# SamsungLabs/nb-asr

Hardware: AMD Instinct MI355X
Metric: utterances_per_sec (higher is better)
Workload: dtype f32

## Files before the change

### nb_asr_amd/csrc/layernorm.hip

```cpp
#include "storage.h"

namespace nbasr {

constexpr int LN_ROWS = 16;
constexpr int LN_QS = 16;

template <typename T, bool MINMAX = false, int FR = Chunk<T>::FR>
__device__ __forceinline__ void tile_statistics(const T* x, int channels, int ld, float eps, size_t base, bool active,
                                                int row, int ql, float (*s_mean)[LN_QS * FR], float (*s_m2)[LN_QS * FR],
                                                float* s_cnt, float* s_mu, float* s_rstd,
                                                float (*s_lo)[LN_QS * FR] = nullptr, float (*s_hi)[LN_QS * FR] = nullptr)
{
    float shift[FR], s1[FR], s2[FR], lo[FR], hi[FR];
#pragma unroll
    for (int r = 0; r < FR; ++r) { shift[r] = 0.f; s1[r] = 0.f; s2[r] = 0.f; lo[r] = 3.0e38f; hi[r] = -3.0e38f; }
    int n = 0;
    if (active && row < channels) {
        load_frames<FR>(x + base + static_cast<size_t>(row) * ld, shift);
        auto fold = [&](const float (&e)[FR]) {
#pragma unroll
            for (int r = 0; r < FR; ++r) {
                const float d = e[r] - shift[r];
                s1[r] += d;
                s2[r] = __builtin_fmaf(d, d, s2[r]);
                if (MINMAX) { lo[r] = fminf(lo[r], e[r]); hi[r] = fmaxf(hi[r], e[r]); }
            }
            ++n;
        };
        int c = row;
        for (; c + 7 * LN_ROWS < channels; c += 8 * LN_ROWS) {
            float e[8][FR];
#pragma unroll
            for (int u = 0; u < 8; ++u) load_frames<FR>(x + base + static_cast<size_t>(c + u * LN_ROWS) * ld, e[u]);
#pragma unroll
            for (int u = 0; u < 8; ++u) fold(e[u]);
        }
        for (; c + 3 * LN_ROWS < channels; c += 4 * LN_ROWS) {
            float e[4][FR];
#pragma unroll
            for (int u = 0; u < 4; ++u) load_frames<FR>(x + base + static_cast<size_t>(c + u * LN_ROWS) * ld, e[u]);
#pragma unroll
            for (int u = 0; u < 4; ++u) fold(e[u]);
        }
        for (; c < channels; c += LN_ROWS) {
            float e[FR];
            load_frames<FR>(x + base + static_cast<size_t>(c) * ld, e);
            fold(e);
        }
    }
    const float fn = static_cast<float>(n);
#pragma unroll
    for (int r = 0; r < FR; ++r) {
        const float dm = n ? s1[r] / fn : 0.f;
        s_mean[row][ql * FR + r] = shift[r] + dm;
        s_m2[row][ql * FR + r] = n ? fmaxf(s2[r] - dm * s1[r], 0.f) : 0.f;
        if (MINMAX) { s_lo[row][ql * FR + r] = lo[r]; s_hi[row][ql * FR + r] = hi[r]; }
    }
    if (ql == 0) s_cnt[row] = fn;
    __syncthreads();

    if (threadIdx.x < LN_QS * FR) {
        const int col = threadIdx.x;
        float cnt = 0.f, mean = 0.f, m2 = 0.f;
#pragma unroll
        for (int k = 0; k < LN_ROWS; ++k) {
            const float nb = s_cnt[k];
            if (nb > 0.f) {
                const float tot = cnt + nb;
                const float delta = s_mean[k][col] - mean;
                mean += delta * (nb / tot);
                m2 += s_m2[k][col] + delta * delta * (cnt * nb / tot);
                cnt = tot;
            }
        }
        s_mu[col] = mean;
        s_rstd[col] = 1.0f / sqrtf(m2 / fmaxf(cnt, 1.f) + eps);
        if (MINMAX) {
            float l = s_lo[0][col], h = s_hi[0][col];
#pragma unroll
            for (int k = 1; k < LN_ROWS; ++k) { l = fminf(l, s_lo[k][col]); h = fmaxf(h, s_hi[k][col]); }
            s_lo[0][col] = l; s_hi[0][col] = h;
        }
    }
    __syncthreads();
}

template <typename TI, typename TO, bool ABSMAX>
__global__ __launch_bounds__(256) void layernorm_channels_kernel(
    const TI* x, const float* __restrict__ gamma, const float* __restrict__ beta,
    TO* y, int channels, int frames, int ld, float eps, unsigned* __restrict__ absmax)
{
    constexpr int FR = Chunk<TI>::FR;
    __shared__ float s_mean[LN_ROWS][LN_QS * FR];
    __shared__ float s_m2[LN_ROWS][LN_QS * FR];
    __shared__ float s_cnt[LN_ROWS];
    __shared__ float s_mu[LN_QS * FR];
    __shared__ float s_rstd[LN_QS * FR];

    const int ql = threadIdx.x & (LN_QS - 1);
    const int row = threadIdx.x / LN_QS;
    const int nq = ld / FR;
    const int q = blockIdx.x * LN_QS + ql;
    const int b = blockIdx.y;
    const bool active = q < nq;
    const size_t base = static_cast<size_t>(b) * channels * ld + static_cast<size_t>(q) * FR;

    tile_statistics<TI>(x, channels, ld, eps, base, active, row, ql, s_mean, s_m2, s_cnt, s_mu, s_rstd);

    if (!active && !ABSMAX) return;
    float mu[FR], rs[FR];
#pragma unroll
    for (int r = 0; r < FR; ++r) { mu[r] = s_mu[ql * FR + r]; rs[r] = s_rstd[ql * FR + r]; }
    const int t0 = q * FR;
    float amax = 0.f;
    for (int c = row; active && c < channels; c += LN_ROWS) {
        const size_t off = base + static_cast<size_t>(c) * ld;
        float o[FR];
        load_frames<FR>(x + off, o);
        const float g = gamma[c], bt = beta[c];
#pragma unroll
        for (int r = 0; r < FR; ++r) {
            o[r] = (o[r] - mu[r]) * rs[r] * g + bt;
            if (t0 + r >= frames) o[r] = 0.f;
            if (ABSMAX) amax = fmaxf(amax, finite_abs(o[r]));
        }
        store_frames<FR, false>(y + off, o);
    }
    if (ABSMAX) {
#pragma unroll
        for (int m = 32; m >= 1; m >>= 1) amax = fmaxf(amax, __shfl_xor(amax, m));
        if ((threadIdx.x & 63) == 0) atomicMax(absmax + b, __float_as_uint(amax));
    }
}

template <typename T>
__global__ __launch_bounds__(256) void channel_stats_kernel(const T* __restrict__ x, float* __restrict__ stats,
                                                            int channels, int frames, int ld, float eps)
{
    constexpr int FR = Chunk<T>::FR;
    __shared__ float s_mean[LN_ROWS][LN_QS * FR];
    __shared__ float s_m2[LN_ROWS][LN_QS * FR];
    __shared__ float s_cnt[LN_ROWS];
    __shared__ float s_mu[LN_QS * FR];
    __shared__ float s_rstd[LN_QS * FR];

    const int ql = threadIdx.x & (LN_QS - 1);
    const int row = threadIdx.x / LN_QS;
    const int nq = ld / FR;
    const int q = blockIdx.x * LN_QS + ql;
    const int b = blockIdx.y;
    const bool active = q < nq;
    const size_t base = static_cast<size_t>(b) * channels * ld + static_cast<size_t>(q) * FR;

    tile_statistics<T>(x, channels, ld, eps, base, active, row, ql, s_mean, s_m2, s_cnt, s_mu, s_rstd);

    if (threadIdx.x < LN_QS * FR) {
        const int t = blockIdx.x * (LN_QS * FR) + threadIdx.x;
        if (t < ld) {
            const bool live = t < frames;
            float* srow = stats + static_cast<size_t>(b) * 2 * ld;
            srow[t] = live ? s_mu[threadIdx.x] : 0.f;
            srow[ld + t] = live ? s_rstd[threadIdx.x] : 0.f;
        }
    }
}

}

using namespace nbasr;

static int layernorm_impl(const char* what, const void* x, const float* gamma, const float* beta, void* y, float* absmax,
                          int batch, int channels, int frames, int ld, float eps, nbasr_stream_t stream,
                          int in_dtype = NBASR_F32, int out_dtype = NBASR_F32)
{
    clear_error();
    NBASR_REQUIRE((in_dtype == NBASR_F32 || in_dtype == NBASR_BF16) && (out_dtype == NBASR_F32 || out_dtype == NBASR_BF16) &&
                  !(in_dtype == NBASR_F32 && out_dtype == NBASR_BF16), NBASR_EINVAL,
                  "%s: storage types (%d -> %d) unsupported (f32 -> f32, bf16 -> bf16, bf16 -> f32)", what, in_dtype, out_dtype);
    NBASR_REQUIRE(batch >= 0 && channels > 0 && frames >= 0, NBASR_EINVAL, "%s: bad sizes", what);
    const int fr = in_dtype == NBASR_BF16 ? 8 : 4;
    NBASR_REQUIRE(ld >= frames && ld % fr == 0, NBASR_EALIGN, "%s: ld=%d must be >= frames=%d and a multiple of %d", what, ld, frames, fr);
    if (batch == 0 || ld == 0) return NBASR_OK;
    NBASR_REQUIRE(x && gamma && beta && y, NBASR_ENULL, "%s: NULL pointer", what);
    NBASR_REQUIRE(aligned16(x) && aligned16(y), NBASR_EALIGN, "%s: x, y must be 16-byte aligned", what);
    NBASR_REQUIRE(batch <= 65535, NBASR_EINVAL, "%s: batch %d > 65535", what, batch);
    NBASR_REQUIRE(!absmax || in_dtype == NBASR_F32, NBASR_EINVAL, "%s: the absmax by-product exists for fp32 tensors only", what);
    const int nq = ld / fr;
    const dim3 grid((nq + LN_QS - 1) / LN_QS, batch);
    if (in_dtype == NBASR_BF16) {
        if (out_dtype == NBASR_BF16)
            hipLaunchKernelGGL((layernorm_channels_kernel<bf16_t, bf16_t, false>), grid, dim3(256), 0, as_stream(stream),
                               static_cast<const bf16_t*>(x), gamma, beta, static_cast<bf16_t*>(y), channels, frames, ld, eps, static_cast<unsigned*>(nullptr));
        else
            hipLaunchKernelGGL((layernorm_channels_kernel<bf16_t, float, false>), grid, dim3(256), 0, as_stream(stream),
                               static_cast<const bf16_t*>(x), gamma, beta, static_cast<float*>(y), channels, frames, ld, eps, static_cast<unsigned*>(nullptr));
    } else if (absmax) {
        zero_async(absmax, sizeof(float) * batch, as_stream(stream));
        hipLaunchKernelGGL((layernorm_channels_kernel<float, float, true>), grid, dim3(256), 0, as_stream(stream),
                           static_cast<const float*>(x), gamma, beta, static_cast<float*>(y), channels, frames, ld, eps, reinterpret_cast<unsigned*>(absmax));
    } else {
        hipLaunchKernelGGL((layernorm_channels_kernel<float, float, false>), grid, dim3(256), 0, as_stream(stream),
                           static_cast<const float*>(x), gamma, beta, static_cast<float*>(y), channels, frames, ld, eps, static_cast<unsigned*>(nullptr));
    }
    return launch_status(what);
}

extern "C" int nbasr_layernorm_channels(const void* x, const float* gamma, const float* beta, void* y, float* absmax, int batch,
                                        int channels, int frames, int ld, float eps, int in_dtype, int out_dtype, nbasr_stream_t stream)
{
    clear_error();
    NBASR_REQUIRE(!absmax || (in_dtype == NBASR_F32 && out_dtype == NBASR_F32), NBASR_EINVAL,
                  "nbasr_layernorm_channels: the max|y| by-product exists for fp32 -> fp32 only");
    return layernorm_impl("nbasr_layernorm_channels", x, gamma, beta, y, absmax, batch, channels, frames, ld, eps, stream, in_dtype, out_dtype);
}

__global__ __launch_bounds__(256) void channel_stats_bound_kernel(const float* __restrict__ x, const float* __restrict__ gamma,
                                                                  const float* __restrict__ beta, float* __restrict__ stats,
                                                                  unsigned* __restrict__ bound, int channels, int frames, int ld, float eps)
{
    __shared__ float s_mean[LN_ROWS][LN_QS * 4];
    __shared__ float s_m2[LN_ROWS][LN_QS * 4];
    __shared__ float s_cnt[LN_ROWS];
    __shared__ float s_mu[LN_QS * 4];
    __shared__ float s_rstd[LN_QS * 4];
    __shared__ float s_gb[8];
    __shared__ float s_lo[LN_ROWS][LN_QS * 4];
    __shared__ float s_hi[LN_ROWS][LN_QS * 4];

    const int ql = threadIdx.x & (LN_QS - 1);
    const int row = threadIdx.x / LN_QS;
    const int nq = ld >> 2;
    const int q = blockIdx.x * LN_QS + ql;
    const int b = blockIdx.y;
    const bool active = q < nq;
    const size_t base = static_cast<size_t>(b) * channels * ld + static_cast<size_t>(q) * 4;

    float gm = 0.f, bm = 0.f;
    for (int c = threadIdx.x; c < channels; c += 256) { gm = fmaxf(gm, fabsf(gamma[c])); bm = fmaxf(bm, fabsf(beta[c])); }
#pragma unroll
    for (int d = 32; d >= 1; d >>= 1) { gm = fmaxf(gm, __shfl_xor(gm, d)); bm = fmaxf(bm, __shfl_xor(bm, d)); }
    if ((threadIdx.x & 63) == 0) { s_gb[threadIdx.x >> 6] = gm; s_gb[4 + (threadIdx.x >> 6)] = bm; }

    tile_statistics<float, true>(x, channels, ld, eps, base, active, row, ql, s_mean, s_m2, s_cnt, s_mu, s_rstd, s_lo, s_hi);
    gm = fmaxf(fmaxf(s_gb[0], s_gb[1]), fmaxf(s_gb[2], s_gb[3]));
    bm = fmaxf(fmaxf(s_gb[4], s_gb[5]), fmaxf(s_gb[6], s_gb[7]));

    float dev = 0.f;
    if (threadIdx.x < LN_QS * 4) {
        const int t = blockIdx.x * (LN_QS * 4) + threadIdx.x;
        if (t < ld) {
            const bool live = t < frames;
            float* srow = stats + static_cast<size_t>(b) * 2 * ld;
            srow[t] = live ? s_mu[threadIdx.x] : 0.f;
            srow[ld + t] = live ? s_rstd[threadIdx.x] : 0.f;
            if (live) dev = finite_abs(fmaxf(s_hi[0][threadIdx.x] - s_mu[threadIdx.x], s_mu[threadIdx.x] - s_lo[0][threadIdx.x]) * s_rstd[threadIdx.x]);
        }
    }
    if (threadIdx.x < 64) {
#pragma unroll
        for (int d = 32; d >= 1; d >>= 1) dev = fmaxf(dev, __shfl_xor(dev, d));
        if (threadIdx.x == 0) atomicMax(bound + b, __float_as_uint(finite_abs((dev * gm + bm) * 1.0001f)));
    }
}

template <bool NORM>
__global__ __launch_bounds__(256) void normalize_split_kernel(const float* __restrict__ x, const float* __restrict__ stats,
                                                              const float* __restrict__ gamma, const float* __restrict__ beta,
                                                              const float* __restrict__ bound, unsigned char* __restrict__ image,
                                                              int channels, int , int ld,
                                                              int bound_stride)
{
    typedef _Float16 halfx8 __attribute__((ext_vector_type(8)));
    constexpr int SPLIT_PITCH = 68;
    __shared__ __attribute__((aligned(16))) unsigned char s_tile[4][2][4 * SPLIT_PITCH * 16];
    const int ql = threadIdx.x & 63, wv = threadIdx.x >> 6, oct0 = wv + 4 * blockIdx.z;
    const int nq = ld >> 2;
    const int q = blockIdx.x * 64 + ql;
    const int b = blockIdx.y;
    const int n_groups = (channels + 15) >> 4;
    const size_t rows = static_cast<size_t>(ld) + 1;
    unsigned char* const img_b = image + static_cast<size_t>(b) * n_groups * 4 * rows * 16;
    if (blockIdx.x == 0 && blockIdx.z == 0) {
        const uint4 z = make_uint4(0u, 0u, 0u, 0u);
        for (int pl = threadIdx.x; pl < n_groups * 4; pl += 256) *reinterpret_cast<uint4*>(img_b + static_cast<size_t>(pl) * rows * 16) = z;
    }
    if (blockIdx.x * 64 >= nq) return;
    const bool inside = q < nq;
    float scale = 1.f;
    {
        const unsigned bits = __float_as_uint(bound[static_cast<size_t>(b) * bound_stride]);
        const int e = static_cast<int>((bits >> 23) & 0xffu);
        int k = (bits & 0x7fffffffu) ? (127 + 14) - e : 0;
        k = k > 126 ? 126 : (k < -126 ? -126 : k);
        scale = __uint_as_float(static_cast<unsigned>(127 + k) << 23);
    }
    float m4[4] = {0.f, 0.f, 0.f, 0.f}, r4[4] = {0.f, 0.f, 0.f, 0.f};
    if constexpr (NORM) {
        if (inside) {
            const float* st = stats + static_cast<size_t>(b) * 2 * ld + q * 4;
            const float4 mu = *reinterpret_cast<const float4*>(st), rs = *reinterpret_cast<const float4*>(st + ld);
            m4[0] = mu.x; m4[1] = mu.y; m4[2] = mu.z; m4[3] = mu.w;
            r4[0] = rs.x; r4[1] = rs.y; r4[2] = rs.z; r4[3] = rs.w;
        }
    }
    const float* xb = x + static_cast<size_t>(b) * channels * ld + static_cast<size_t>(q) * 4;
    const int n_oct = (channels + 7) >> 3;
    const int oct_step = 4 * gridDim.z;
    auto load_octet = [&](int oct, float4 (&t)[8]) {
#pragma unroll
        for (int c = 0; c < 8; ++c) {
            const int ch = oct * 8 + c;
            t[c] = make_float4(0.f, 0.f, 0.f, 0.f);
            if (inside && oct < n_oct && ch < channels) t[c] = *reinterpret_cast<const float4*>(xb + static_cast<size_t>(ch) * ld);
        }
    };
    unsigned char* const tile_hi = s_tile[wv][0];
    unsigned char* const tile_lo = s_tile[wv][1];
    float4 cur[8];
    if (oct0 < 2 * n_groups) load_octet(oct0, cur);
    for (int oct = oct0; oct < 2 * n_groups; oct += oct_step) {
        float4 nxt[8];
        if (oct + oct_step < 2 * n_groups) load_octet(oct + oct_step, nxt);
        else {
#pragma unroll
            for (int c = 0; c < 8; ++c) nxt[c] = make_float4(0.f, 0.f, 0.f, 0.f);
        }
        float v[8][4];
#pragma unroll
        for (int c = 0; c < 8; ++c) {
            const int ch = oct * 8 + c;
            float g = 0.f, be = 0.f;
            if constexpr (NORM) {
                if (oct < n_oct && ch < channels) { g = gamma[ch]; be = beta[ch]; }
            }
            const float e4[4] = {cur[c].x, cur[c].y, cur[c].z, cur[c].w};
#pragma unroll
            for (int r = 0; r < 4; ++r) {
                if constexpr (NORM) v[c][r] = (ch < channels) ? ln_apply(e4[r], m4[r], r4[r], g, be) * scale : 0.f;
                else                v[c][r] = e4[r] * scale;
            }
        }
#pragma unroll
        for (int r = 0; r < 4; ++r) {
            halfx8 hi, lo;
#pragma unroll
            for (int c = 0; c < 8; ++c) {
                const _Float16 h = static_cast<_Float16>(v[c][r]);
                hi[c] = h;
                lo[c] = static_cast<_Float16>(v[c][r] - static_cast<float>(h));
            }
            *reinterpret_cast<halfx8*>(tile_hi + (r * SPLIT_PITCH + ql) * 16) = hi;
            *reinterpret_cast<halfx8*>(tile_lo + (r * SPLIT_PITCH + ql) * 16) = lo;
        }
        asm volatile("s_waitcnt lgkmcnt(0)" ::: "memory");
        unsigned char* plane_hi = img_b + ((static_cast<size_t>(oct >> 1) * 4 + (oct & 1)) * rows + 1 + static_cast<size_t>(blockIdx.x) * 256) * 16;
        unsigned char* plane_lo = plane_hi + 2 * rows * 16;
#pragma unroll
        for (int k = 0; k < 4; ++k) {
            const int src = ((ql & 3) * SPLIT_PITCH + 16 * k + (ql >> 2)) * 16;
            const halfx8 hi = *reinterpret_cast<const halfx8*>(tile_hi + src);
            const halfx8 lo = *reinterpret_cast<const halfx8*>(tile_lo + src);
            const int f = 64 * k + ql;
            if (blockIdx.x * 256 + f < ld) {
                *reinterpret_cast<halfx8*>(plane_hi + f * 16) = hi;
                *reinterpret_cast<halfx8*>(plane_lo + f * 16) = lo;
            }
        }
        asm volatile("s_waitcnt lgkmcnt(0)" ::: "memory");
#pragma unroll
        for (int c = 0; c < 8; ++c) cur[c] = nxt[c];
    }
}

static int split_grid_z(int tiles, int batch)
{
    const long long wgs = static_cast<long long>(tiles) * batch;
    int z = 4;
    while (z < 16 && wgs * z < 512) z *= 2;
    return z;
}

extern "C" int nbasr_layernorm_split_image(const float* x, const float* gamma, const float* beta, float* stats, float* bound,
                                           void* image, int batch, int channels, int frames, int ld, float eps,
                                           nbasr_stream_t stream)
{
    clear_error();
    NBASR_REQUIRE(batch >= 0 && channels > 0 && frames >= 0, NBASR_EINVAL, "nbasr_layernorm_split_image: bad sizes");
    NBASR_REQUIRE(ld >= frames && ld % 4 == 0, NBASR_EALIGN, "nbasr_layernorm_split_image: ld=%d must be >= frames=%d and a multiple of 4", ld, frames);
    if (batch == 0 || ld == 0) return NBASR_OK;
    NBASR_REQUIRE(x && gamma && beta && stats && bound && image, NBASR_ENULL, "nbasr_layernorm_split_image: NULL pointer");
    NBASR_REQUIRE(aligned16(x) && aligned16(stats) && aligned16(image), NBASR_EALIGN, "nbasr_layernorm_split_image: x, stats, image must be 16-byte aligned");
    NBASR_REQUIRE(batch <= 65535, NBASR_EINVAL, "nbasr_layernorm_split_image: batch %d > 65535", batch);
    zero_async(bound, sizeof(float) * batch, as_stream(stream));
    const int nq = ld / 4;
    hipLaunchKernelGGL(channel_stats_bound_kernel, dim3((nq + LN_QS - 1) / LN_QS, batch), dim3(256), 0, as_stream(stream),
                       x, gamma, beta, stats, reinterpret_cast<unsigned*>(bound), channels, frames, ld, eps);
    hipLaunchKernelGGL(normalize_split_kernel<true>, dim3((nq + 63) / 64, batch, split_grid_z((nq + 63) / 64, batch)), dim3(256), 0, as_stream(stream),
                       x, stats, gamma, beta, bound, static_cast<unsigned char*>(image), channels, frames, ld, 1);
    return launch_status("nbasr_layernorm_split_image");
}

__global__ __launch_bounds__(256) void input_range_kernel(const float* __restrict__ x, unsigned* __restrict__ range,
                                                          int channels, int frames, int ld)
{
    __shared__ float s_max[4][256];
    __shared__ unsigned s_bad[4];
    const int b = blockIdx.y;
    const int lane = threadIdx.x & 63, slice = threadIdx.x >> 6;
    const int t0 = (blockIdx.x * 64 + lane) * 4;
    float m[4] = {0.f, 0.f, 0.f, 0.f};
    unsigned bad = 0u;
    if (t0 < frames) {
        const float* col = x + static_cast<size_t>(b) * channels * ld + t0;
        const bool whole = t0 + 4 <= ld && ld % 4 == 0 && (reinterpret_cast<size_t>(x) & 15) == 0;
        for (int c = slice; c < channels; c += 4) {
            float v[4] = {0.f, 0.f, 0.f, 0.f};
            if (whole) {
                const float4 q = *reinterpret_cast<const float4*>(col + static_cast<size_t>(c) * ld);
                v[0] = q.x; v[1] = q.y; v[2] = q.z; v[3] = q.w;
            } else {
#pragma unroll
                for (int r = 0; r < 4; ++r) if (t0 + r < frames) v[r] = col[static_cast<size_t>(c) * ld + r];
            }
#pragma unroll
            for (int r = 0; r < 4; ++r) {
                const float a = fabsf(v[r]);
                if (t0 + r < frames) {
                    if (!(a <= 3.4028234664e38f)) bad = 1u;
                    else m[r] = fmaxf(m[r], a);
                }
            }
        }
    }
#pragma unroll
    for (int r = 0; r < 4; ++r) s_max[slice][lane * 4 + r] = m[r];
#pragma unroll
    for (int d = 32; d >= 1; d >>= 1) bad |= __shfl_xor(bad, d);
    if (lane == 0) s_bad[slice] = bad;
    __syncthreads();
    const int t = blockIdx.x * 256 + threadIdx.x;
    const float fmax_ = fmaxf(fmaxf(s_max[0][threadIdx.x], s_max[1][threadIdx.x]), fmaxf(s_max[2][threadIdx.x], s_max[3][threadIdx.x]));
    float hi = fmax_, lo = (t < frames && fmax_ > 0.f) ? fmax_ : __uint_as_float(0x7f800000u);
#pragma unroll
    for (int d = 32; d >= 1; d >>= 1) {
        hi = fmaxf(hi, __shfl_xor(hi, d));
        lo = fminf(lo, __shfl_xor(lo, d));
    }
    if (lane == 0) {
        atomicMax(range + 4 * b, __float_as_uint(hi));
        atomicMin(range + 4 * b + 1, __float_as_uint(lo));
        if (slice == 0 && (s_bad[0] | s_bad[1] | s_bad[2] | s_bad[3])) atomicOr(range + 4 * b + 2, 0x3f800000u);
    }
}

__global__ void input_range_init_kernel(unsigned* __restrict__ range, int batch)
{
    const int b = blockIdx.x * blockDim.x + threadIdx.x;
    if (b < batch) { range[4 * b] = 0u; range[4 * b + 1] = 0x7f800000u; range[4 * b + 2] = 0u; range[4 * b + 3] = 0u; }
}

extern "C" int nbasr_input_range(const float* x, float* range, int batch, int channels, int frames, int ld, nbasr_stream_t stream)
{
    clear_error();
    NBASR_REQUIRE(batch >= 0 && channels > 0 && frames >= 0 && ld >= frames, NBASR_EINVAL, "nbasr_input_range: bad sizes");
    if (batch == 0) return NBASR_OK;
    NBASR_REQUIRE(range, NBASR_ENULL, "nbasr_input_range: range is NULL");
    NBASR_REQUIRE(batch <= 65535, NBASR_EINVAL, "nbasr_input_range: batch %d > 65535", batch);
    hipLaunchKernelGGL(input_range_init_kernel, dim3((batch + 255) / 256), dim3(256), 0, as_stream(stream), reinterpret_cast<unsigned*>(range), batch);
    if (frames > 0) {
        NBASR_REQUIRE(x, NBASR_ENULL, "nbasr_input_range: x is NULL");
        hipLaunchKernelGGL(input_range_kernel, dim3((frames + 255) / 256, batch), dim3(256), 0, as_stream(stream), x,
                           reinterpret_cast<unsigned*>(range), channels, frames, ld);
    }
    return launch_status("nbasr_input_range");
}

extern "C" int nbasr_split_image_ranged(const float* x, const float* x_range, void* image, int batch, int channels, int frames,
                                        int ld, nbasr_stream_t stream)
{
    clear_error();
    NBASR_REQUIRE(batch >= 0 && channels > 0 && frames >= 0, NBASR_EINVAL, "nbasr_split_image_ranged: bad sizes");
    NBASR_REQUIRE(ld >= frames && ld % 4 == 0, NBASR_EALIGN, "nbasr_split_image_ranged: ld=%d must be >= frames=%d and a multiple of 4", ld, frames);
    if (batch == 0 || ld == 0) return NBASR_OK;
    NBASR_REQUIRE(x && x_range && image, NBASR_ENULL, "nbasr_split_image_ranged: NULL pointer");
    NBASR_REQUIRE(aligned16(x) && aligned16(image), NBASR_EALIGN, "nbasr_split_image_ranged: x, image must be 16-byte aligned");
    NBASR_REQUIRE(batch <= 65535, NBASR_EINVAL, "nbasr_split_image_ranged: batch %d > 65535", batch);
    const int nq = ld / 4;
    hipLaunchKernelGGL(normalize_split_kernel<false>, dim3((nq + 63) / 64, batch, split_grid_z((nq + 63) / 64, batch)), dim3(256), 0, as_stream(stream),
                       x, static_cast<const float*>(nullptr), static_cast<const float*>(nullptr), static_cast<const float*>(nullptr),
                       x_range, static_cast<unsigned char*>(image), channels, frames, ld, 4);
    return launch_status("nbasr_split_image_ranged");
}

extern "C" int nbasr_channel_stats(const void* x, float* stats, int batch, int channels, int frames, int ld, float eps, int dtype,
                                     nbasr_stream_t stream)
{
    clear_error();
    NBASR_REQUIRE(dtype == NBASR_F32 || dtype == NBASR_BF16, NBASR_EINVAL, "nbasr_channel_stats: unknown dtype %d", dtype);
    NBASR_REQUIRE(batch >= 0 && channels > 0 && frames >= 0, NBASR_EINVAL, "nbasr_channel_stats: bad sizes");
    const int fr = dtype == NBASR_BF16 ? 8 : 4;
    NBASR_REQUIRE(ld >= frames && ld % fr == 0, NBASR_EALIGN, "nbasr_channel_stats: ld=%d must be >= frames=%d and a multiple of %d", ld, frames, fr);
    if (batch == 0 || ld == 0) return NBASR_OK;
    NBASR_REQUIRE(x && stats, NBASR_ENULL, "nbasr_channel_stats: NULL pointer");
    NBASR_REQUIRE(aligned16(x) && aligned16(stats), NBASR_EALIGN, "nbasr_channel_stats: x, stats must be 16-byte aligned");
    NBASR_REQUIRE(batch <= 65535, NBASR_EINVAL, "nbasr_channel_stats: batch %d > 65535", batch);
    const int nq = ld / fr;
    const dim3 grid((nq + LN_QS - 1) / LN_QS, batch);
    if (dtype == NBASR_BF16)
        hipLaunchKernelGGL(channel_stats_kernel<bf16_t>, grid, dim3(256), 0, as_stream(stream), static_cast<const bf16_t*>(x), stats, channels, frames, ld, eps);
    else
        hipLaunchKernelGGL(channel_stats_kernel<float>, grid, dim3(256), 0, as_stream(stream), static_cast<const float*>(x), stats, channels, frames, ld, eps);
    return launch_status("nbasr_channel_stats");
}

template <typename T, bool NORM>
__global__ __launch_bounds__(256) void bf16_image_kernel(const T* __restrict__ x, const float* __restrict__ stats,
                                                         const float* __restrict__ gamma, const float* __restrict__ beta,
                                                         unsigned char* __restrict__ image, int channels, int frames, int ld)
{
    constexpr int FR = Chunk<T>::FR;
    const int ql = threadIdx.x & 15, oct0 = threadIdx.x >> 4;
    const int nq = ld / FR;
    const int q = blockIdx.x * 16 + ql;
    const int b = blockIdx.y;
    const int n_groups = (channels + 15) >> 4;
    const size_t rows = static_cast<size_t>(ld) + 1;
    unsigned char* const img_b = image + static_cast<size_t>(b) * n_groups * 2 * rows * 16;
    if (blockIdx.x == 0) {
        const uint4 z = make_uint4(0u, 0u, 0u, 0u);
        for (int pl = threadIdx.x; pl < n_groups * 2; pl += 256) *reinterpret_cast<uint4*>(img_b + static_cast<size_t>(pl) * rows * 16) = z;
    }
    if (q >= nq) return;
    float m[FR], r[FR];
#pragma unroll
    for (int e = 0; e < FR; ++e) { m[e] = 0.f; r[e] = 1.f; }
    if (NORM) {
        const float* st = stats + static_cast<size_t>(b) * 2 * ld + q * FR;
        load_frames<FR>(st, m);
        load_frames<FR>(st + ld, r);
    }
    const T* xb = x + static_cast<size_t>(b) * channels * ld + static_cast<size_t>(q) * FR;
    const int n_oct = (channels + 7) >> 3;
    for (int oct = oct0; oct < 2 * n_groups; oct += 16) {
        float v[8][FR];
#pragma unroll
        for (int c = 0; c < 8; ++c) {
            const int ch = oct * 8 + c;
#pragma unroll
            for (int e = 0; e < FR; ++e) v[c][e] = 0.f;
            if (oct < n_oct && ch < channels) {
                load_frames<FR>(xb + static_cast<size_t>(ch) * ld, v[c]);
                if (NORM) {
                    const float g = gamma[ch], be = beta[ch];
#pragma unroll
// ... 79 lines not shown
```

### nb_asr_amd/csrc/lstm.hip

```cpp
#include "common.h"

#include <cstdlib>
#include <mutex>
#include <vector>

namespace nbasr {

constexpr int NBASR_MAX_DEVICES = 64;

typedef float floatx4 __attribute__((ext_vector_type(4)));

int lstm_input_projection(const float* x, const float* w_ih, const float* b_ih, const float* b_hh, float* gates,
                          int batch, int c_in, int frames, int ld, int rows4h, LnRef ln, hipStream_t stream);

__device__ __forceinline__ float sigmoidf_(float v) { return 1.0f / (1.0f + expf(-v)); }

constexpr int LSTM_WAVES = 8;
constexpr int LSTM_CHUNKS = 4;

constexpr int LSTMP_HU = 8;

__global__ __launch_bounds__(256) void lstm_pack_whh_kernel(const float* __restrict__ w_hh, float4* __restrict__ packed, int hidden,
                                                            int slices, int kchunks_p)
{
// ... 4 lines not shown
        const int mt = e % 2; e /= 2;
        const int kc = e % kchunks_p; e /= kchunks_p;
        const int slice = static_cast<int>(e);
        const int unit = slice * LSTMP_HU + mt * 4 + ((lane & 15) >> 2), gate = lane & 3, k = kc * 16 + (lane >> 4) * 4;
        float4 v = make_float4(0.f, 0.f, 0.f, 0.f);
        if (unit < hidden && k < hidden) v = *reinterpret_cast<const float4*>(w_hh + (static_cast<size_t>(gate) * hidden + unit) * hidden + k);
        packed[i] = v;
    }
}

__global__ __launch_bounds__(64 * LSTM_WAVES) void lstm_step_packed_kernel(
    const float* __restrict__ gates_in,
    const float4* __restrict__ wp,
    float* __restrict__ cell, float* h_out, int batch, int frames, int hidden, int kchunks_p, int t, int prio)
{
    __shared__ float red[LSTM_WAVES][2][4][64];
    if (prio) __builtin_amdgcn_s_setprio(3);

    const int lane = threadIdx.x & 63, wave = threadIdx.x >> 6;
    const int i16 = lane & 15, kq = lane >> 4;
    const int j0 = blockIdx.x * LSTMP_HU, b0 = blockIdx.y * 16;

    const int jj = threadIdx.x & 7, bb = (threadIdx.x >> 3) & 15;
    const int ej = j0 + jj, eb = b0 + bb;
    const bool e_ok = threadIdx.x < 128 && ej < hidden && eb < batch;
    float pre[4] = {0.f, 0.f, 0.f, 0.f};
    float c_prev = 0.f;
    if (e_ok) {
        const float* gin = gates_in + (static_cast<size_t>(t) * batch + eb) * (4 * hidden);
#pragma unroll
        for (int g = 0; g < 4; ++g) pre[g] = gin[g * hidden + ej];
        if (t > 0) c_prev = cell[static_cast<size_t>(eb) * hidden + ej];
    }

    floatx4 acc[2] = {floatx4{0.f, 0.f, 0.f, 0.f}, floatx4{0.f, 0.f, 0.f, 0.f}};
    if (t > 0) {
        const bool col_ok = (b0 + i16) < batch;
        const float* hrow = h_out + (static_cast<size_t>(b0 + i16) * frames + (t - 1)) * hidden;
        const float4* wslice = wp + static_cast<size_t>(blockIdx.x) * kchunks_p * 2 * 64 + lane;
        for (int base = wave * LSTM_CHUNKS; base < kchunks_p; base += LSTM_WAVES * LSTM_CHUNKS) {
            float4 hv[LSTM_CHUNKS], wv[LSTM_CHUNKS][2];
#pragma unroll
            for (int c = 0; c < LSTM_CHUNKS; ++c) {
                const int k = (base + c) * 16 + kq * 4;
                hv[c] = make_float4(0.f, 0.f, 0.f, 0.f);
                if (col_ok && k < hidden) hv[c] = *reinterpret_cast<const float4*>(hrow + k);
                wv[c][0] = wslice[static_cast<size_t>(base + c) * 2 * 64];
                wv[c][1] = wslice[static_cast<size_t>(base + c) * 2 * 64 + 64];
            }
#pragma unroll
            for (int c = 0; c < LSTM_CHUNKS; ++c) {
#pragma unroll
                for (int m = 0; m < 2; ++m) acc[m] = __builtin_amdgcn_mfma_f32_16x16x4f32(wv[c][m].x, hv[c].x, acc[m], 0, 0, 0);
#pragma unroll
                for (int m = 0; m < 2; ++m) acc[m] = __builtin_amdgcn_mfma_f32_16x16x4f32(wv[c][m].y, hv[c].y, acc[m], 0, 0, 0);
#pragma unroll
                for (int m = 0; m < 2; ++m) acc[m] = __builtin_amdgcn_mfma_f32_16x16x4f32(wv[c][m].z, hv[c].z, acc[m], 0, 0, 0);
#pragma unroll
                for (int m = 0; m < 2; ++m) acc[m] = __builtin_amdgcn_mfma_f32_16x16x4f32(wv[c][m].w, hv[c].w, acc[m], 0, 0, 0);
            }
        }
    }
#pragma unroll
    for (int m = 0; m < 2; ++m)
#pragma unroll
        for (int r = 0; r < 4; ++r) red[wave][m][r][lane] = acc[m][r];
    __syncthreads();

    if (!e_ok) return;
    const int mt = jj >> 2, pl = (jj & 3) * 16 + bb;
#pragma unroll
    for (int g = 0; g < 4; ++g) {
        float s = red[0][mt][g][pl];
#pragma unroll
        for (int w = 1; w < LSTM_WAVES; ++w) s += red[w][mt][g][pl];
        pre[g] += s;
    }
    const float c_new = sigmoidf_(pre[1]) * c_prev + sigmoidf_(pre[0]) * tanhf(pre[2]);
    const float h_new = sigmoidf_(pre[3]) * tanhf(c_new);
    cell[static_cast<size_t>(eb) * hidden + ej] = c_new;
    h_out[(static_cast<size_t>(eb) * frames + t) * hidden + ej] = h_new;
}

template <bool BCT>
__global__ __launch_bounds__(256) void head_kernel(
    const float* __restrict__ h, const float* __restrict__ w, const float* __restrict__ bias,
    float* __restrict__ out, int rows, int features, int classes, int frames, int ld, const LnRef ln)
{
    const int lane = threadIdx.x & 63, wave = threadIdx.x >> 6;
    const int i16 = lane & 15, kq = lane >> 4;
    const int r0 = (blockIdx.x * 4 + wave) * 16;
    if (r0 >= rows) return;

    floatx4 acc[4], part[4];
#pragma unroll
    for (int n = 0; n < 4; ++n) { acc[n] = floatx4{0.f, 0.f, 0.f, 0.f}; part[n] = floatx4{0.f, 0.f, 0.f, 0.f}; }

    const int row = r0 + i16;
    const bool row_ok = row < rows;
    const int kchunks = (features + 15) / 16;
    for (int c = 0; c < kchunks; ++c) {
        if ((c & 7) == 0 && c) {
#pragma unroll
            for (int n = 0; n < 4; ++n) { acc[n] += part[n]; part[n] = floatx4{0.f, 0.f, 0.f, 0.f}; }
        }
        const int k = c * 16 + kq * 4;
        const bool kok = k < features;
        float av[4] = {0.f, 0.f, 0.f, 0.f};
        if (row_ok && kok) {
            if (!BCT) {
                const float4 v = *reinterpret_cast<const float4*>(h + static_cast<size_t>(row) * features + k);
                av[0] = v.x; av[1] = v.y; av[2] = v.z; av[3] = v.w;
            } else {
                const int bb = row / frames, tt = row - bb * frames;
                const float* p = h + (static_cast<size_t>(bb) * features + k) * ld + tt;
#pragma unroll
                for (int e = 0; e < 4; ++e) av[e] = p[static_cast<size_t>(e) * ld];
                if (ln.stats) {
                    const float* st = ln.stats + static_cast<size_t>(bb) * 2 * ld;
                    const float mean = st[tt], rstd = st[ld + tt];
#pragma unroll
                    for (int e = 0; e < 4; ++e) av[e] = ln_apply(av[e], mean, rstd, ln.gamma[k + e], ln.beta[k + e]);
                }
            }
        }
#pragma unroll
        for (int n = 0; n < 4; ++n) {
            const int cls = n * 16 + i16;
            float4 wv = make_float4(0.f, 0.f, 0.f, 0.f);
            if (cls < classes && kok) wv = *reinterpret_cast<const float4*>(w + static_cast<size_t>(cls) * features + k);
            part[n] = __builtin_amdgcn_mfma_f32_16x16x4f32(av[0], wv.x, part[n], 0, 0, 0);
            part[n] = __builtin_amdgcn_mfma_f32_16x16x4f32(av[1], wv.y, part[n], 0, 0, 0);
            part[n] = __builtin_amdgcn_mfma_f32_16x16x4f32(av[2], wv.z, part[n], 0, 0, 0);
            part[n] = __builtin_amdgcn_mfma_f32_16x16x4f32(av[3], wv.w, part[n], 0, 0, 0);
        }
    }
#pragma unroll
    for (int n = 0; n < 4; ++n) acc[n] += part[n];
#pragma unroll
    for (int n = 0; n < 4; ++n) {
        const int cls = n * 16 + i16;
        if (cls >= classes) continue;
        const float bv = bias[cls];
#pragma unroll
        for (int r = 0; r < 4; ++r) {
            const int rr = r0 + kq * 4 + r;
            if (rr < rows) out[static_cast<size_t>(rr) * classes + cls] = acc[n][r] + bv;
        }
    }
}

constexpr int LSTMS_QUADS = LSTM_WAVES * LSTM_CHUNKS * 4;
constexpr int LSTMS_IMAGE_FLOATS = LSTMS_QUADS * 16 * 4;
constexpr int LSTMS_HEADER_WORDS = 64;
constexpr unsigned long long LSTMS_TIMEOUT_TICKS = 100000000ull;

typedef unsigned lstm_u4 __attribute__((ext_vector_type(4)));

__device__ __forceinline__ unsigned lstm_tag(int t) { return (static_cast<unsigned>((t >> 1) + 1) & 1u) << 30; }

__global__ __launch_bounds__(64 * LSTM_WAVES) void lstm_seq_kernel(
    const float* __restrict__ gates_in,
    const float4* __restrict__ wp,
    float* __restrict__ cell, float* __restrict__ h_out, unsigned* status, float* hx,
    int batch, int frames, int hidden, int kchunks_p, int flags)
{
    __shared__ float4 red[2][LSTM_WAVES][2][64];
    __shared__ int stop;
    if ((flags & NBASR_LSTM_SEQ_INJECT_FAULT) && blockIdx.x == 0) return;

    const int lane = threadIdx.x & 63, wave = __builtin_amdgcn_readfirstlane(threadIdx.x >> 6);
    const int i16 = lane & 15, kq = lane >> 4;
    const int slice = blockIdx.x, tile = blockIdx.y;
    const int b0 = tile * 16;
    if (threadIdx.x == 0) stop = 0;

    float4 wv[LSTM_CHUNKS][2];
    {
        const bool mine = wave * LSTM_CHUNKS < kchunks_p;
        const float4* wslice = wp + (static_cast<size_t>(slice) * kchunks_p + (mine ? wave * LSTM_CHUNKS : 0)) * 2 * 64 + lane;
#pragma unroll
        for (int c = 0; c < LSTM_CHUNKS; ++c) {
            wv[c][0] = mine ? wslice[c * 128] : make_float4(0.f, 0.f, 0.f, 0.f);
            wv[c][1] = mine ? wslice[c * 128 + 64] : make_float4(0.f, 0.f, 0.f, 0.f);
        }
    }

    const int eu = slice * LSTMP_HU + (wave & 1) * 4 + kq, eb = b0 + i16;
    const bool e_ok = eu < hidden && eb < batch;
    const size_t gate_off = static_cast<size_t>(min(eb, batch - 1)) * (4 * hidden) + min(eu, hidden - 1);
    const int quad = slice * 2 + (wave & 1);
    const bool q_ok = kq == 0 && quad * 4 < hidden && eb < batch;
    float c_state = 0.f;

    float* const image = hx + static_cast<size_t>(tile) * 2 * LSTMS_IMAGE_FLOATS;
    const __amdgpu_buffer_rsrc_t hxr = __builtin_amdgcn_make_buffer_rsrc(image, 0, 2 * LSTMS_IMAGE_FLOATS * 4, 0x00020000);
    bool live[LSTM_CHUNKS];
#pragma unroll
    for (int c = 0; c < LSTM_CHUNKS; ++c) live[c] = eb < batch && ((wave * LSTM_CHUNKS + c) * 4 + kq) * 4 < hidden;
    __syncthreads();

    int t = 0;
    for (; t < frames; ++t) {
        float pre[4];
        {
            const float* gin = gates_in + static_cast<size_t>(t) * batch * (4 * hidden) + gate_off;
#pragma unroll
            for (int g = 0; g < 4; ++g) pre[g] = gin[g * hidden];
        }
        floatx4 acc[2] = {floatx4{0.f, 0.f, 0.f, 0.f}, floatx4{0.f, 0.f, 0.f, 0.f}};
        if (t > 0) {
            const int img = ((t - 1) & 1) * LSTMS_QUADS;
            const unsigned want = lstm_tag(t - 1);
            floatx4 hr[LSTM_CHUNKS];
            const unsigned long long t_start = __builtin_amdgcn_s_memrealtime();
            bool ok = false;
            for (;;) {
#pragma unroll
                for (int c = 0; c < LSTM_CHUNKS; ++c) {
// ... 288 lines not shown
```

Baseline: 11470.

## Widen layernorm stat/range kernels and stage head weights through shared memory

The channel statistics/bound kernel grows to 512 threads covering 32 quads per block, with a flattened 1D grid of batch times tiles. The input-range kernel grows to 1024 threads with 16 channel slices and an 8-way unrolled float4 load loop. The classifier head kernel now double-buffers weight tiles in LDS and prefetches activations and weights one k-block ahead. All three changes aim to raise memory-level parallelism and cut redundant global weight loads. In exchange they use more registers and LDS, and the head kernel gains an extra __syncthreads per k-block.

```diff
diff --git a/nb_asr_amd/csrc/layernorm.hip b/nb_asr_amd/csrc/layernorm.hip
--- a/nb_asr_amd/csrc/layernorm.hip
+++ b/nb_asr_amd/csrc/layernorm.hip
@@ -5,11 +5,11 @@
 constexpr int LN_ROWS = 16;
 constexpr int LN_QS = 16;
 
-template <typename T, bool MINMAX = false, int FR = Chunk<T>::FR>
+template <typename T, bool MINMAX = false, int FR = Chunk<T>::FR, int QS = LN_QS>
 __device__ __forceinline__ void tile_statistics(const T* x, int channels, int ld, float eps, size_t base, bool active,
-                                                int row, int ql, float (*s_mean)[LN_QS * FR], float (*s_m2)[LN_QS * FR],
+                                                int row, int ql, float (*s_mean)[QS * FR], float (*s_m2)[QS * FR],
                                                 float* s_cnt, float* s_mu, float* s_rstd,
-                                                float (*s_lo)[LN_QS * FR] = nullptr, float (*s_hi)[LN_QS * FR] = nullptr)
+                                                float (*s_lo)[QS * FR] = nullptr, float (*s_hi)[QS * FR] = nullptr)
 {
     float shift[FR], s1[FR], s2[FR], lo[FR], hi[FR];
 #pragma unroll
@@ -59,7 +59,7 @@
     if (ql == 0) s_cnt[row] = fn;
     __syncthreads();
 
-    if (threadIdx.x < LN_QS * FR) {
+    if (threadIdx.x < QS * FR) {
         const int col = threadIdx.x;
         float cnt = 0.f, mean = 0.f, m2 = 0.f;
 #pragma unroll
@@ -214,53 +214,57 @@
     return layernorm_impl("nbasr_layernorm_channels", x, gamma, beta, y, absmax, batch, channels, frames, ld, eps, stream, in_dtype, out_dtype);
 }
 
-__global__ __launch_bounds__(256) void channel_stats_bound_kernel(const float* __restrict__ x, const float* __restrict__ gamma,
-                                                                  const float* __restrict__ beta, float* __restrict__ stats,
-                                                                  unsigned* __restrict__ bound, int channels, int frames, int ld, float eps)
-{
-    __shared__ float s_mean[LN_ROWS][LN_QS * 4];
-    __shared__ float s_m2[LN_ROWS][LN_QS * 4];
+constexpr int LN_BOUND_QS = 32;
+constexpr int LN_BOUND_THREADS = LN_BOUND_QS * LN_ROWS;
+constexpr int LN_BOUND_WAVES = LN_BOUND_THREADS / 64;
+
+__global__ __launch_bounds__(LN_BOUND_THREADS) void channel_stats_bound_kernel(const float* __restrict__ x, const float* __restrict__ gamma,
+                                                                               const float* __restrict__ beta, float* __restrict__ stats,
+                                                                               unsigned* __restrict__ bound, int batch, int channels, int frames, int ld, float eps)
+{
+    constexpr int COLS = LN_BOUND_QS * 4;
+    __shared__ float s_mean[LN_ROWS][COLS];
+    __shared__ float s_m2[LN_ROWS][COLS];
     __shared__ float s_cnt[LN_ROWS];
-    __shared__ float s_mu[LN_QS * 4];
-    __shared__ float s_rstd[LN_QS * 4];
-    __shared__ float s_gb[8];
-    __shared__ float s_lo[LN_ROWS][LN_QS * 4];
-    __shared__ float s_hi[LN_ROWS][LN_QS * 4];
-
-    const int ql = threadIdx.x & (LN_QS - 1);
-    const int row = threadIdx.x / LN_QS;
+    __shared__ float s_mu[COLS];
+    __shared__ float s_rstd[COLS];
+    __shared__ float s_gb[2][LN_BOUND_WAVES];
+    __shared__ float s_lo[LN_ROWS][COLS];
+    __shared__ float s_hi[LN_ROWS][COLS];
+
+    const int ql = threadIdx.x & (LN_BOUND_QS - 1);
+    const int row = threadIdx.x / LN_BOUND_QS;
     const int nq = ld >> 2;
-    const int q = blockIdx.x * LN_QS + ql;
-    const int b = blockIdx.y;
+    const int b = blockIdx.x % batch, tile = blockIdx.x / batch;
+    const int q = tile * LN_BOUND_QS + ql;
     const bool active = q < nq;
     const size_t base = static_cast<size_t>(b) * channels * ld + static_cast<size_t>(q) * 4;
 
     float gm = 0.f, bm = 0.f;
-    for (int c = threadIdx.x; c < channels; c += 256) { gm = fmaxf(gm, fabsf(gamma[c])); bm = fmaxf(bm, fabsf(beta[c])); }
+    for (int c = threadIdx.x; c < channels; c += LN_BOUND_THREADS) { gm = fmaxf(gm, fabsf(gamma[c])); bm = fmaxf(bm, fabsf(beta[c])); }
 #pragma unroll
     for (int d = 32; d >= 1; d >>= 1) { gm = fmaxf(gm, __shfl_xor(gm, d)); bm = fmaxf(bm, __shfl_xor(bm, d)); }
-    if ((threadIdx.x & 63) == 0) { s_gb[threadIdx.x >> 6] = gm; s_gb[4 + (threadIdx.x >> 6)] = bm; }
-
-    tile_statistics<float, true>(x, channels, ld, eps, base, active, row, ql, s_mean, s_m2, s_cnt, s_mu, s_rstd, s_lo, s_hi);
-    gm = fmaxf(fmaxf(s_gb[0], s_gb[1]), fmaxf(s_gb[2], s_gb[3]));
-    bm = fmaxf(fmaxf(s_gb[4], s_gb[5]), fmaxf(s_gb[6], s_gb[7]));
-
+    if ((threadIdx.x & 63) == 0) { s_gb[0][threadIdx.x >> 6] = gm; s_gb[1][threadIdx.x >> 6] = bm; }
+
+    tile_statistics<float, true, 4, LN_BOUND_QS>(x, channels, ld, eps, base, active, row, ql, s_mean, s_m2, s_cnt, s_mu, s_rstd, s_lo, s_hi);
+
+    if (threadIdx.x >= COLS) return;
+    const int t = tile * COLS + threadIdx.x;
+    if (t - static_cast<int>(threadIdx.x & 63) >= ld) return;
+    gm = s_gb[0][0]; bm = s_gb[1][0];
+#pragma unroll
+    for (int k = 1; k < LN_BOUND_WAVES; ++k) { gm = fmaxf(gm, s_gb[0][k]); bm = fmaxf(bm, s_gb[1][k]); }
     float dev = 0.f;
-    if (threadIdx.x < LN_QS * 4) {
-        const int t = blockIdx.x * (LN_QS * 4) + threadIdx.x;
-        if (t < ld) {
-            const bool live = t < frames;
-            float* srow = stats + static_cast<size_t>(b) * 2 * ld;
-            srow[t] = live ? s_mu[threadIdx.x] : 0.f;
-            srow[ld + t] = live ? s_rstd[threadIdx.x] : 0.f;
-            if (live) dev = finite_abs(fmaxf(s_hi[0][threadIdx.x] - s_mu[threadIdx.x], s_mu[threadIdx.x] - s_lo[0][threadIdx.x]) * s_rstd[threadIdx.x]);
-        }
-    }
-    if (threadIdx.x < 64) {
-#pragma unroll
-        for (int d = 32; d >= 1; d >>= 1) dev = fmaxf(dev, __shfl_xor(dev, d));
-        if (threadIdx.x == 0) atomicMax(bound + b, __float_as_uint(finite_abs((dev * gm + bm) * 1.0001f)));
-    }
+    if (t < ld) {
+        const bool live = t < frames;
+        float* srow = stats + static_cast<size_t>(b) * 2 * ld;
+        srow[t] = live ? s_mu[threadIdx.x] : 0.f;
+        srow[ld + t] = live ? s_rstd[threadIdx.x] : 0.f;
+        if (live) dev = finite_abs(fmaxf(s_hi[0][threadIdx.x] - s_mu[threadIdx.x], s_mu[threadIdx.x] - s_lo[0][threadIdx.x]) * s_rstd[threadIdx.x]);
+    }
+#pragma unroll
+    for (int d = 32; d >= 1; d >>= 1) dev = fmaxf(dev, __shfl_xor(dev, d));
+    if ((threadIdx.x & 63) == 0) atomicMax(bound + b, __float_as_uint(finite_abs((dev * gm + bm) * 1.0001f)));
 }
 
 template <bool NORM>
@@ -393,35 +397,32 @@
     NBASR_REQUIRE(batch <= 65535, NBASR_EINVAL, "nbasr_layernorm_split_image: batch %d > 65535", batch);
     zero_async(bound, sizeof(float) * batch, as_stream(stream));
     const int nq = ld / 4;
-    hipLaunchKernelGGL(channel_stats_bound_kernel, dim3((nq + LN_QS - 1) / LN_QS, batch), dim3(256), 0, as_stream(stream),
-                       x, gamma, beta, stats, reinterpret_cast<unsigned*>(bound), channels, frames, ld, eps);
+    hipLaunchKernelGGL(channel_stats_bound_kernel, dim3(static_cast<unsigned>((nq + LN_BOUND_QS - 1) / LN_BOUND_QS) * batch), dim3(LN_BOUND_THREADS), 0, as_stream(stream),
+                       x, gamma, beta, stats, reinterpret_cast<unsigned*>(bound), batch, channels, frames, ld, eps);
     hipLaunchKernelGGL(normalize_split_kernel<true>, dim3((nq + 63) / 64, batch, split_grid_z((nq + 63) / 64, batch)), dim3(256), 0, as_stream(stream),
                        x, stats, gamma, beta, bound, static_cast<unsigned char*>(image), channels, frames, ld, 1);
     return launch_status("nbasr_layernorm_split_image");
 }
 
-__global__ __launch_bounds__(256) void input_range_kernel(const float* __restrict__ x, unsigned* __restrict__ range,
-                                                          int channels, int frames, int ld)
-{
-    __shared__ float s_max[4][256];
-    __shared__ unsigned s_bad[4];
-    const int b = blockIdx.y;
-    const int lane = threadIdx.x & 63, slice = threadIdx.x >> 6;
-    const int t0 = (blockIdx.x * 64 + lane) * 4;
+constexpr int IR_LANES = 64;
+constexpr int IR_SLICES = 16;
+constexpr int IR_THREADS = IR_LANES * IR_SLICES;
+constexpr int IR_FRAMES = IR_LANES * 4;
+
+__global__ __launch_bounds__(IR_THREADS) void input_range_kernel(const float* __restrict__ x, unsigned* __restrict__ range,
+                                                                 int channels, int frames, int ld)
+{
+    __shared__ float s_max[IR_SLICES][IR_FRAMES];
+    __shared__ unsigned s_bad[IR_THREADS / 64];
+    const int b = blockIdx.y, tile = blockIdx.x;
+    const int lane = threadIdx.x & (IR_LANES - 1), slice = threadIdx.x / IR_LANES;
+    const int t0 = (tile * IR_LANES + lane) * 4;
     float m[4] = {0.f, 0.f, 0.f, 0.f};
     unsigned bad = 0u;
     if (t0 < frames) {
         const float* col = x + static_cast<size_t>(b) * channels * ld + t0;
         const bool whole = t0 + 4 <= ld && ld % 4 == 0 && (reinterpret_cast<size_t>(x) & 15) == 0;
-        for (int c = slice; c < channels; c += 4) {
-            float v[4] = {0.f, 0.f, 0.f, 0.f};
-            if (whole) {
-                const float4 q = *reinterpret_cast<const float4*>(col + static_cast<size_t>(c) * ld);
-                v[0] = q.x; v[1] = q.y; v[2] = q.z; v[3] = q.w;
-            } else {
-#pragma unroll
-                for (int r = 0; r < 4; ++r) if (t0 + r < frames) v[r] = col[static_cast<size_t>(c) * ld + r];
-            }
+        auto fold = [&](const float (&v)[4]) {
 #pragma unroll
             for (int r = 0; r < 4; ++r) {
                 const float a = fabsf(v[r]);
@@ -430,26 +431,54 @@
                     else m[r] = fmaxf(m[r], a);
                 }
             }
+        };
+        if (whole) {
+            for (int c = slice; c < channels; c += 8 * IR_SLICES) {
+                float4 q[8];
+#pragma unroll
+                for (int u = 0; u < 8; ++u) {
+                    q[u] = make_float4(0.f, 0.f, 0.f, 0.f);
+                    if (c + u * IR_SLICES < channels) q[u] = *reinterpret_cast<const float4*>(col + static_cast<size_t>(c + u * IR_SLICES) * ld);
+                }
+#pragma unroll
+                for (int u = 0; u < 8; ++u) {
+                    const float v[4] = {q[u].x, q[u].y, q[u].z, q[u].w};
+                    fold(v);
+                }
+            }
+        } else {
+            for (int c = slice; c < channels; c += IR_SLICES) {
+                float v[4] = {0.f, 0.f, 0.f, 0.f};
+#pragma unroll
+                for (int r = 0; r < 4; ++r) if (t0 + r < frames) v[r] = col[static_cast<size_t>(c) * ld + r];
+                fold(v);
+            }
         }
     }
 #pragma unroll
     for (int r = 0; r < 4; ++r) s_max[slice][lane * 4 + r] = m[r];
 #pragma unroll
     for (int d = 32; d >= 1; d >>= 1) bad |= __shfl_xor(bad, d);
-    if (lane == 0) s_bad[slice] = bad;
+    if ((threadIdx.x & 63) == 0) s_bad[threadIdx.x >> 6] = bad;
     __syncthreads();
-    const int t = blockIdx.x * 256 + threadIdx.x;
-    const float fmax_ = fmaxf(fmaxf(s_max[0][threadIdx.x], s_max[1][threadIdx.x]), fmaxf(s_max[2][threadIdx.x], s_max[3][threadIdx.x]));
+    if (threadIdx.x >= IR_FRAMES) return;
+    const int t = tile * IR_FRAMES + threadIdx.x;
+    float fmax_ = s_max[0][threadIdx.x];
+#pragma unroll
+    for (int k = 1; k < IR_SLICES; ++k) fmax_ = fmaxf(fmax_, s_max[k][threadIdx.x]);
     float hi = fmax_, lo = (t < frames && fmax_ > 0.f) ? fmax_ : __uint_as_float(0x7f800000u);
 #pragma unroll
     for (int d = 32; d >= 1; d >>= 1) {
         hi = fmaxf(hi, __shfl_xor(hi, d));
         lo = fminf(lo, __shfl_xor(lo, d));
     }
-    if (lane == 0) {
+    if ((threadIdx.x & 63) == 0) {
         atomicMax(range + 4 * b, __float_as_uint(hi));
         atomicMin(range + 4 * b + 1, __float_as_uint(lo));
-        if (slice == 0 && (s_bad[0] | s_bad[1] | s_bad[2] | s_bad[3])) atomicOr(range + 4 * b + 2, 0x3f800000u);
+        unsigned any = 0u;
+#pragma unroll
+        for (int k = 0; k < IR_THREADS / 64; ++k) any |= s_bad[k];
+        if (threadIdx.x == 0 && any) atomicOr(range + 4 * b + 2, 0x3f800000u);
     }
 }
 
@@ -469,7 +498,7 @@
     hipLaunchKernelGGL(input_range_init_kernel, dim3((batch + 255) / 256), dim3(256), 0, as_stream(stream), reinterpret_cast<unsigned*>(range), batch);
     if (frames > 0) {
         NBASR_REQUIRE(x, NBASR_ENULL, "nbasr_input_range: x is NULL");
-        hipLaunchKernelGGL(input_range_kernel, dim3((frames + 255) / 256, batch), dim3(256), 0, as_stream(stream), x,
+        hipLaunchKernelGGL(input_range_kernel, dim3((frames + IR_FRAMES - 1) / IR_FRAMES, batch), dim3(IR_THREADS), 0, as_stream(stream), x,
                            reinterpret_cast<unsigned*>(range), channels, frames, ld);
     }
     return launch_status("nbasr_input_range");
diff --git a/nb_asr_amd/csrc/lstm.hip b/nb_asr_amd/csrc/lstm.hip
--- a/nb_asr_amd/csrc/lstm.hip
+++ b/nb_asr_amd/csrc/lstm.hip
@@ -110,15 +110,18 @@
     h_out[(static_cast<size_t>(eb) * frames + t) * hidden + ej] = h_new;
 }
 
+constexpr int HEAD_KB = 8;
+
 template <bool BCT>
 __global__ __launch_bounds__(256) void head_kernel(
     const float* __restrict__ h, const float* __restrict__ w, const float* __restrict__ bias,
     float* __restrict__ out, int rows, int features, int classes, int frames, int ld, const LnRef ln)
 {
+    __shared__ float4 s_w[2][HEAD_KB][4][64];
     const int lane = threadIdx.x & 63, wave = threadIdx.x >> 6;
     const int i16 = lane & 15, kq = lane >> 4;
     const int r0 = (blockIdx.x * 4 + wave) * 16;
-    if (r0 >= rows) return;
+    const bool wave_live = r0 < rows;
 
     floatx4 acc[4], part[4];
 #pragma unroll
@@ -127,42 +130,82 @@
     const int row = r0 + i16;
     const bool row_ok = row < rows;
     const int kchunks = (features + 15) / 16;
-    for (int c = 0; c < kchunks; ++c) {
-        if ((c & 7) == 0 && c) {
+    const int kblocks = (kchunks + HEAD_KB - 1) / HEAD_KB;
+    const int stage_cls = wave * 16 + i16;
+    const bool stage_ok = stage_cls < classes;
+
+    const float* hrow = h;
+    const float* wrow = w + (stage_ok ? static_cast<size_t>(stage_cls) * features : 0);
+    float mean = 0.f, rstd = 0.f;
+    if (row_ok) {
+        if (!BCT) {
+            hrow = h + static_cast<size_t>(row) * features;
+        } else {
+            const int bb = row / frames, tt = row - bb * frames;
+            hrow = h + static_cast<size_t>(bb) * features * ld + tt;
+            if (ln.stats) {
+                const float* st = ln.stats + static_cast<size_t>(bb) * 2 * ld;
+                mean = st[tt]; rstd = st[ld + tt];
+            }
+        }
+    }
+    float hn[HEAD_KB][4];
+    float4 wn[HEAD_KB];
+    auto fetch = [&](int kb) {
+#pragma unroll
+        for (int cc = 0; cc < HEAD_KB; ++cc) {
+            int k = (kb * HEAD_KB + cc) * 16 + kq * 4;
+            k = k < features ? k : features - 4;
+            if (!BCT) {
+                const float4 v = *reinterpret_cast<const float4*>(hrow + k);
+                hn[cc][0] = v.x; hn[cc][1] = v.y; hn[cc][2] = v.z; hn[cc][3] = v.w;
+            } else {
+                const float* p = hrow + static_cast<size_t>(k) * ld;
+#pragma unroll
+                for (int e = 0; e < 4; ++e) hn[cc][e] = p[static_cast<size_t>(e) * ld];
+                if (ln.stats) {
+#pragma unroll
+                    for (int e = 0; e < 4; ++e) hn[cc][e] = ln_apply(hn[cc][e], mean, rstd, ln.gamma[k + e], ln.beta[k + e]);
+                }
+            }
+            wn[cc] = *reinterpret_cast<const float4*>(wrow + k);
+        }
+    };
+
+    fetch(0);
+    for (int kb = 0; kb < kblocks; ++kb) {
+        float4 (*sw)[4][64] = s_w[kb & 1];
+        float av[HEAD_KB][4];
+#pragma unroll
+        for (int cc = 0; cc < HEAD_KB; ++cc) {
+            const bool kok = (kb * HEAD_KB + cc) * 16 + kq * 4 < features;
+            sw[cc][wave][lane] = (stage_ok && kok) ? wn[cc] : make_float4(0.f, 0.f, 0.f, 0.f);
+#pragma unroll
+            for (int e = 0; e < 4; ++e) av[cc][e] = (row_ok && kok) ? hn[cc][e] : 0.f;
+        }
+        if (kb + 1 < kblocks) fetch(kb + 1);
+        __syncthreads();
+        if (!wave_live) continue;
+        if (kb) {
 #pragma unroll
             for (int n = 0; n < 4; ++n) { acc[n] += part[n]; part[n] = floatx4{0.f, 0.f, 0.f, 0.f}; }
         }
-        const int k = c * 16 + kq * 4;
-        const bool kok = k < features;
-        float av[4] = {0.f, 0.f, 0.f, 0.f};
-        if (row_ok && kok) {
-            if (!BCT) {
-                const float4 v = *reinterpret_cast<const float4*>(h + static_cast<size_t>(row) * features + k);
-                av[0] = v.x; av[1] = v.y; av[2] = v.z; av[3] = v.w;
-            } else {
-                const int bb = row / frames, tt = row - bb * frames;
-                const float* p = h + (static_cast<size_t>(bb) * features + k) * ld + tt;
-#pragma unroll
-                for (int e = 0; e < 4; ++e) av[e] = p[static_cast<size_t>(e) * ld];
-                if (ln.stats) {
-                    const float* st = ln.stats + static_cast<size_t>(bb) * 2 * ld;
-                    const float mean = st[tt], rstd = st[ld + tt];
-#pragma unroll
-                    for (int e = 0; e < 4; ++e) av[e] = ln_apply(av[e], mean, rstd, ln.gamma[k + e], ln.beta[k + e]);
-                }
-            }
-        }
-#pragma unroll
-        for (int n = 0; n < 4; ++n) {
-            const int cls = n * 16 + i16;
-            float4 wv = make_float4(0.f, 0.f, 0.f, 0.f);
-            if (cls < classes && kok) wv = *reinterpret_cast<const float4*>(w + static_cast<size_t>(cls) * features + k);
-            part[n] = __builtin_amdgcn_mfma_f32_16x16x4f32(av[0], wv.x, part[n], 0, 0, 0);
-            part[n] = __builtin_amdgcn_mfma_f32_16x16x4f32(av[1], wv.y, part[n], 0, 0, 0);
-            part[n] = __builtin_amdgcn_mfma_f32_16x16x4f32(av[2], wv.z, part[n], 0, 0, 0);
-            part[n] = __builtin_amdgcn_mfma_f32_16x16x4f32(av[3], wv.w, part[n], 0, 0, 0);
-        }
-    }
+#pragma unroll
+        for (int cc = 0; cc < HEAD_KB; ++cc) {
+            if (kb * HEAD_KB + cc >= kchunks) break;
+            float4 wv[4];
+#pragma unroll
+            for (int n = 0; n < 4; ++n) wv[n] = sw[cc][n][lane];
+#pragma unroll
+            for (int n = 0; n < 4; ++n) {
+                part[n] = __builtin_amdgcn_mfma_f32_16x16x4f32(av[cc][0], wv[n].x, part[n], 0, 0, 0);
+                part[n] = __builtin_amdgcn_mfma_f32_16x16x4f32(av[cc][1], wv[n].y, part[n], 0, 0, 0);
+                part[n] = __builtin_amdgcn_mfma_f32_16x16x4f32(av[cc][2], wv[n].z, part[n], 0, 0, 0);
+                part[n] = __builtin_amdgcn_mfma_f32_16x16x4f32(av[cc][3], wv[n].w, part[n], 0, 0, 0);
+            }
+        }
+    }
+    if (!wave_live) return;
 #pragma unroll
     for (int n = 0; n < 4; ++n) acc[n] += part[n];
 #pragma unroll
```

Result: no change. 11460 (-0.1%).
